# nelpy/ghost

Measured on NVIDIA B200. Metric: cwt_output_coeffs_per_sec, higher is better.
Workload: dtype f32

## Files before the change

ghost_b200/csrc/cabi.cu:

```cuda
#include "plan.h"
#include "common.cuh"
#include <cstring>
#include <cstdio>
#include <cstdlib>
#include <new>

namespace gcwt {

static thread_local std::string g_last_error;
static thread_local int64_t g_launches = 0;

void set_error(const std::string& msg) { g_last_error = msg; }
void count_launch(int n) { g_launches += n; }
int64_t launches_so_far() { return g_launches; }

int prof_begin(gcwt_plan* p, int kind, cudaStream_t st, int tag) {
    if (!p->profile) return -1;
    gcwt_plan::Span sp;
    sp.kind = kind;
    sp.tag = tag;
    sp.launches = (int)g_launches;
    if (cudaEventCreate(&sp.a) != cudaSuccess || cudaEventCreate(&sp.b) != cudaSuccess) return -1;
    cudaEventRecord(sp.a, st);
    p->spans.push_back(sp);
// ... 120 lines not shown
        sc.n_terms = d->n_terms[s];
        sc.term_off = off;
        sc.level = -2;
        if (sc.L < 1 || sc.n_terms < 1 || sc.k_first < 0 || sc.k_first + sc.n_terms > sc.L) {
            set_error("plan_create: inconsistent scale " + std::to_string(s));
            delete p;
            return GCWT_ERR_ARG;
        }
        off += sc.n_terms;
        p->scales.push_back(sc);
    }
    p->terms.assign(d->terms, d->terms + off);

    int rc = GCWT_OK;
    {
        cudaError_t e = cudaMalloc((void**)&p->d_scales, sizeof(ScaleInfo) * p->n_scales);
        if (e == cudaSuccess) e = cudaMalloc((void**)&p->d_terms, sizeof(double) * p->terms.size());
        if (e == cudaSuccess) e = cudaMemcpy(p->d_scales, p->scales.data(), sizeof(ScaleInfo) * p->n_scales, cudaMemcpyHostToDevice);
        if (e == cudaSuccess) e = cudaMemcpy(p->d_terms, p->terms.data(), sizeof(double) * p->terms.size(), cudaMemcpyHostToDevice);
        if (e != cudaSuccess) { set_error(std::string("plan_create: ") + cudaGetErrorString(e)); rc = GCWT_ERR_CUDA; }
    }
    if (rc == GCWT_OK) {
        if (p->compute_type == GCWT_F32) rc = fast_plan_build(p);
        else for (int s = 0; s < p->n_scales; ++s) p->generic_ids.push_back(s);
    }
    if (rc == GCWT_OK && p->compute_type == GCWT_F32) {
        cudaError_t e = cudaMemcpy(p->d_scales, p->scales.data(), sizeof(ScaleInfo) * p->n_scales, cudaMemcpyHostToDevice);
        if (e != cudaSuccess) { set_error(std::string("plan_create: ") + cudaGetErrorString(e)); rc = GCWT_ERR_CUDA; }
    }
    if (rc != GCWT_OK) { gcwt_plan_destroy(p); return rc; }
    *out = p;
    return GCWT_OK;
}

int gcwt_plan_destroy(gcwt_plan* p) {
    if (!p) return GCWT_OK;
    DeviceScope dev_scope(p->device);
    prof_collect(p);
    host_stage_free(p);
    fast_plan_free(p);
    if (p->d_scales) cudaFree(p->d_scales);
    if (p->d_terms) cudaFree(p->d_terms);
    if (p->ws.ptr) cudaFree(p->ws.ptr);
    if (p->d_means) cudaFree(p->d_means);
    if (p->d_partial) cudaFree(p->d_partial);
    if (p->d_twiddle) cudaFree(p->d_twiddle);
    if (p->d_tw1k) cudaFree(p->d_tw1k);
    if (p->d_tw_fine) cudaFree(p->d_tw_fine);
    if (p->d_hcache) cudaFree(p->d_hcache);
    for (int k = 0; k < gcwt_plan::kSideStreams; ++k) {
        if (p->side_stream[k]) { cudaStreamSynchronize(p->side_stream[k]); cudaStreamDestroy(p->side_stream[k]); }
        if (p->ev_join[k]) cudaEventDestroy(p->ev_join[k]);
    }
    if (p->ev_fork) cudaEventDestroy(p->ev_fork);
    delete p;
    return GCWT_OK;
}

int gcwt_profile_enable(gcwt_plan* p, int32_t on) {
    if (!p) { set_error("profile_enable: NULL plan"); return GCWT_ERR_ARG; }
    p->profile = on != 0;
    return GCWT_OK;
}

int gcwt_profile_read(gcwt_plan* p, double* ms_out, int64_t* launches_out, int32_t reset) {
    if (!p || !ms_out || !launches_out) { set_error("profile_read: NULL argument"); return GCWT_ERR_ARG; }
    DeviceScope dev_scope(p->device);
    prof_collect(p);
    if (getenv("GCWT_CLASS_TIMES")) {
        for (int t = 0; t < 64; ++t)
            if (p->class_ms[t] > 0) fprintf(stderr, "gcwt class level %d: %.4f ms\n", t - 2, p->class_ms[t]);
    }
    if (reset) for (int t = 0; t < 64; ++t) p->class_ms[t] = 0;
    for (int k = 0; k < GCWT_PROFILE_KINDS; ++k) {
        ms_out[k] = p->prof_ms[k];
        launches_out[k] = p->prof_launches[k];
        if (reset) { p->prof_ms[k] = 0; p->prof_launches[k] = 0; }
    }
    return GCWT_OK;
}

int gcwt_plan_levels(const gcwt_plan* p, int32_t* levels_out) {
    if (!p || !levels_out) { set_error("plan_levels: NULL argument"); return GCWT_ERR_ARG; }
    for (int s = 0; s < p->n_scales; ++s) levels_out[s] = p->scales[s].level;
    return GCWT_OK;
}

size_t gcwt_plan_workspace_bytes(const gcwt_plan* p) { return p ? p->ws.bytes : 0; }

int gcwt_guard_stats(const gcwt_plan* p, int64_t* last_pairs, int64_t* total_pairs, int64_t* checked_pairs,
                     unsigned char* scale_flags) {
    if (!p) { set_error("guard_stats: NULL plan"); return GCWT_ERR_ARG; }
    if (last_pairs) *last_pairs = p->guard_last;
    if (total_pairs) *total_pairs = p->guard_total;
    if (checked_pairs) *checked_pairs = p->guard_checked;
    if (scale_flags)
        for (int s = 0; s < p->n_scales; ++s) scale_flags[s] = (size_t)s < p->guard_last_flags.size() ? p->guard_last_flags[s] : 0;
    return GCWT_OK;
}

int gcwt_channel_means(const void* x, int32_t in_type, int64_t n_channels, int64_t n_samples,
                       int64_t x_stride, double* means_dev, int32_t device, void* stream) {
    if (!x || !means_dev) { set_error("channel_means: NULL argument"); return GCWT_ERR_ARG; }
    if (in_type != GCWT_F32 && in_type != GCWT_F64) { set_error("channel_means: bad in_type"); return GCWT_ERR_ARG; }
    DeviceScope dev_scope(device);
    double* partial = nullptr;
// ... 151 lines not shown
```

ghost_b200/csrc/fast_path.cu:

```cuda
#include "plan.h"
#include "common.cuh"
#include "multiplier.cuh"
#include <algorithm>
#include <atomic>
#include <cmath>
#include <cstdio>
#include <cstdlib>
#include <map>
#include <type_traits>

namespace gcwt {

constexpr int kMaxFastLevel = 14;
constexpr int kMaxFullScales = 64;
constexpr double kMaxHaloFrac = 0.45;

__constant__ float c_halfband[kHalfbandOdd];
constexpr int kSmallCoef = (2 + 4 + 8) * kInterpT;
__constant__ float c_interp_small[kSmallCoef];
constexpr int kWideCoef = (4 + 8) * kWideT;
__constant__ float c_interp_wide[kWideCoef];

static double bessel_i0(double x) {
    double sum = 1.0, term = 1.0;
// ... 567 lines not shown
        }
        *(float4*)(out + (int64_t)c * out_stride + (i0 + j0 - out_lo)) = make_float4(o[0], o[1], o[2], o[3]);
    }
    if (acc != nullptr) {
#pragma unroll
        for (int o = 16; o > 0; o >>= 1) {
            e_out += __shfl_xor_sync(0xffffffffu, e_out, o);
            if (FIRST) e_in += __shfl_xor_sync(0xffffffffu, e_in, o);
        }
        __syncthreads();
        if ((threadIdx.x & 31) == 0) { ev[threadIdx.x >> 5] = e_out; if (FIRST) ev[8 + (threadIdx.x >> 5)] = e_in; }
        __syncthreads();
        if (threadIdx.x == 0) {
            double* a = acc + (int64_t)c * acc_stride;
            float so = 0.f, si = 0.f;
#pragma unroll
            for (int w = 0; w < 8; ++w) { so += ev[w]; if (FIRST) si += ev[8 + w]; }
            if (so != 0.f) atomicAdd(a + level, (double)so);
            if (FIRST && si != 0.f) atomicAdd(a, (double)si);
        }
    }
}

struct FusedParams {
    const void* src;
    int64_t src_stride;
    int64_t src_lo, src_hi;
    const double* means;
    int log2d;
    int p_cols;
    int log2p;
    float inv_nc;
    int64_t offset, hop, n_chunks, n;
    int n_scales;
    const int32_t* scale_ids;
    const float2* table;
    void* out;
    int64_t s_stride, c_stride;
    int iters;
    int units_per_chunk;
    int log2u;
    const float* coef;
    const float2* twf;
    const int32_t* scale_nmu;
    double* acc;
    int acc_stride;
    int class_idx;
    float ech_weight;
    float* pow;
    int pow_stride;
    float pow_weight;
    int guard_every;
    int q_mode;
};

__device__ __forceinline__ float2 tw_pos(const float2* __restrict__ twf, int k) {
    const float2 t = __ldg(twf + (k & (kFullN - 1)));
    return make_float2(t.x, -t.y);
}

__device__ __forceinline__ float sqrt_abs_approx(float v) {
    float r;
    asm("sqrt.approx.ftz.f32 %0, %1;" : "=f"(r) : "f"(fabsf(v)));
    return r;
}

__device__ __forceinline__ float sqrt_approx(float v) {
    float r;
    asm("sqrt.approx.ftz.f32 %0, %1;" : "=f"(r) : "f"(v));
    return r;
}

template <int KIND> struct out_elem { typedef float type; };
template <> struct out_elem<GCWT_OUT_COMPLEX> { typedef float2 type; };

__device__ __forceinline__ void st_pred(float* p, float v, unsigned on) {
#ifdef GCWT_EXP_CSSTORE
    asm volatile("{\n\t.reg .pred q;\n\tsetp.ne.b32 q, %2, 0;\n\t@q st.global.cs.f32 [%0], %1;\n\t}"
                 :: "l"(p), "f"(v), "r"(on) : "memory");
    return;
#endif
    asm volatile("{\n\t.reg .pred q;\n\tsetp.ne.b32 q, %2, 0;\n\t@q st.global.f32 [%0], %1;\n\t}"
                 :: "l"(p), "f"(v), "r"(on) : "memory");
}
__device__ __forceinline__ void st_pred(float2* p, float2 v, unsigned on) {
    asm volatile("{\n\t.reg .pred q;\n\tsetp.ne.b32 q, %3, 0;\n\t@q st.global.v2.f32 [%0], {%1, %2};\n\t}"
                 :: "l"(p), "f"(v.x), "f"(v.y), "r"(on) : "memory");
}

template <int KIND>
__device__ __forceinline__ void store_column(typename out_elem<KIND>::type* __restrict__ op, int64_t stride,
                                             unsigned mask, const float2* a) {
#pragma unroll
    for (int k = 0; k < 16; ++k) {
        const unsigned on = mask & (1u << k);
        if constexpr (KIND == GCWT_OUT_COMPLEX) st_pred(op + k * stride, a[k], on);
        else if constexpr (KIND == GCWT_OUT_AMPLITUDE) st_pred(op + k * stride, sqrt_approx(a[k].x * a[k].x + a[k].y * a[k].y), on);
        else st_pred(op + k * stride, a[k].x * a[k].x + a[k].y * a[k].y, on);
    }
}

__device__ __forceinline__ unsigned valid_mask(int rel, int sh, int lo, int hi) {
    const int step = 1 << sh;
    int k_lo = (lo - rel + step - 1) >> sh;
    int k_hi = (hi - rel + step - 1) >> sh;
    k_lo = max(k_lo, 0);
// ... 764 lines not shown
        for (int i = 0; i < 16; ++i) a[i] = A[(g + 16 * i) * 17 + r];
        dft16<+1>(a);
        float2* e = ex + (g * 16) * 16 + r;
        e[0] = a[0];
#pragma unroll
        for (int k = 1; k < 16; ++k) e[k * 16] = cmul(a[k], tw[k]);
#ifndef GCWT_EXP_NOBAR
        __syncthreads();
#endif
        const float2* e2 = ex + g * 16 + r;
#pragma unroll
        for (int k = 0; k < 16; ++k) a[k] = e2[k * 256];
#ifndef GCWT_EXP_NOPASS2
        dft16<+1>(a);
#endif
#ifdef GCWT_EXP_NOSTORE
        store_column<KIND>(out_c + (int64_t)s_ids[s] * prm.s_stride + rel, 256, mask & 1u, a);
#elif defined(GCWT_EXP_HALFSTORE)
        store_column<KIND>(out_c + (int64_t)s_ids[s] * prm.s_stride + rel, 256, mask & 0x5555u, a);
#elif defined(GCWT_EXP_B16STORE)
        {
            unsigned short* o16 = (unsigned short*)(out_c + (int64_t)s_ids[s] * prm.s_stride) + rel;
#pragma unroll
            for (int k = 0; k < 16; ++k)
                if (mask & (1u << k)) o16[k * 512] = (unsigned short)__float_as_uint(a[k].x * a[k].x + a[k].y * a[k].y);
        }
#elif defined(GCWT_EXP_V2STORE)
        {
            float2* o2 = (float2*)(out_c + (int64_t)s_ids[s] * prm.s_stride) + rel;
#pragma unroll
            for (int k = 0; k < 16; k += 2)
                if (mask & (1u << k)) o2[(k >> 1) * 256] = make_float2(a[k].x * a[k].x + a[k].y * a[k].y, a[k + 1].x * a[k + 1].x + a[k + 1].y * a[k + 1].y);
        }
#elif defined(GCWT_EXP_STSSTORE)
        {
            float* stage = (float*)const_cast<float2*>(Yf);
#pragma unroll
            for (int k = 0; k < 16; ++k) stage[k * 256 + rel] = sqrt_approx(a[k].x * a[k].x + a[k].y * a[k].y);
        }
#elif defined(GCWT_EXP_L2STORE)
        store_column<KIND>((typename out_elem<KIND>::type*)prm.out + (blockIdx.x & 255) * 4096 + rel, 256, mask, a);
#else
        store_column<KIND>(out_c + (int64_t)s_ids[s] * prm.s_stride + rel, 256, mask, a);
#endif
        if (MEASURE) guard_pow_add<false>(a, mask, s_pow + (s & 1));
    }
    if (MEASURE) {
        __syncthreads();
        const int s = prm.n_scales - 1;
        if (tid == 0) atomicAdd(prm.pow + (blockIdx.x / prm.n_chunks) * prm.pow_stride + s_ids[s], s_pow[s & 1] * prm.pow_weight);
    }
}

template <typename TIn, int KIND, bool GUARD>
__global__ void __launch_bounds__(256, 2)
fused_full_kernel(const FusedParams prm) {
    extern __shared__ __align__(16) unsigned char smem_raw[];
    float2* Yf = (float2*)smem_raw;
    float2* ex = Yf + kFullN;
    float2* A = ex + kFullN;
    int* s_ids = (int*)(A + kTileA);
    int* s_nmu = s_ids + kMaxFullScales;
    float* s_pow = (float*)(s_nmu + kMaxFullScales);

    const int tid = threadIdx.x;
    if (tid < 2) s_pow[tid] = 0.f;
    const int r = tid & 15;
    const int g = tid >> 4;
    const int64_t qi = blockIdx.x % prm.n_chunks;
    const int64_t c = blockIdx.x / prm.n_chunks;
    const int64_t q = prm.q_mode == 0 ? qi : (prm.q_mode == 1 ? qi * prm.guard_every : qi + qi / (prm.guard_every - 1) + 1);
    const int64_t t0 = q * prm.hop - prm.offset;

    {
        const TIn* src = (const TIn*)prm.src + c * prm.src_stride;
        const double mu = prm.means[c];
        TIn raw[kFullN / 256];
        unsigned inside = 0;
#pragma unroll
        for (int k = 0; k < kFullN / 256; ++k) {
            const int64_t u = t0 + tid + 256 * k;
            const bool ok = u >= prm.src_lo && u < prm.src_hi;
            raw[k] = ok ? src[u] : (TIn)0;
            inside |= (unsigned)ok << k;
        }
        float val[kFullN / 256];
#pragma unroll
        for (int k = 0; k < kFullN / 256; ++k)
            val[k] = (inside >> k & 1) ? (float)((double)raw[k] - mu) : 0.f;
        const float cm = chunk_mean<kFullN / 256>(val, (float*)ex + 2048);
        if (GUARD)
            chunk_energy_add<kFullN / 256>(val, cm, (float*)ex + 2048, prm.acc + c * prm.acc_stride + kGuardLevels + prm.class_idx,
                                           prm.ech_weight);
#pragma unroll
        for (int k = 0; k < kFullN / 256; ++k) A[tid + 256 * k] = make_float2(val[k] - cm, 0.f);
        __syncthreads();
        smem_fft4096_forward(A, Yf, prm.twf);
    }
    float2 tw[16], tw4k[16];
#pragma unroll
    for (int k = 0; k < 16; ++k) {
        tw[k] = tw_pos(prm.twf, 16 * g * k);
        tw4k[k] = tw_pos(prm.twf, tid * k);
    }
    typedef typename out_elem<KIND>::type OutT;
    const int rel = g * 16 + r;
    const unsigned mask = valid_mask(rel, 8, (int)prm.offset, (int)min(prm.offset + prm.hop, prm.n - t0));
    OutT* const out_c = (OutT*)prm.out + c * prm.c_stride + t0;
    if (tid < prm.n_scales) { s_ids[tid] = prm.scale_ids[tid]; s_nmu[tid] = prm.scale_nmu[tid]; }
    __syncthreads();
    full_scale_loop<KIND, GUARD>(prm, Yf, ex, A, s_ids, s_nmu, s_pow, tw, tw4k, out_c, rel, mask);
}

template <int KIND, int LP, bool GUARD>
static void launch_banded_g(unsigned nblk, cudaStream_t st, const FusedParams& prm) {
    static std::atomic<bool> attr_set[64];
    int dev = 0;
    cudaGetDevice(&dev);
    if (!attr_set[dev & 63]) {
        cudaFuncSetAttribute(fused_banded_kernel<KIND, LP, GUARD>, cudaFuncAttributeMaxDynamicSharedMemorySize, (int)kBandedSmem);
        attr_set[dev & 63] = true;
    }
    fused_banded_kernel<KIND, LP, GUARD><<<nblk, 256, kBandedSmem, st>>>(prm);
}

template <int KIND, int LP>
static void launch_banded_one(unsigned nblk, cudaStream_t st, const FusedParams& prm) {
    if (prm.pow != nullptr) launch_banded_g<KIND, LP, true>(nblk, st, prm);
    else launch_banded_g<KIND, LP, false>(nblk, st, prm);
}

static void launch_banded(int kind, int lp, unsigned nblk, cudaStream_t st, const FusedParams& prm) {
    if (kind == GCWT_OUT_COMPLEX) {
        if (lp == 4) launch_banded_one<GCWT_OUT_COMPLEX, 4>(nblk, st, prm);
        else launch_banded_one<GCWT_OUT_COMPLEX, 0>(nblk, st, prm);
    } else if (kind == GCWT_OUT_AMPLITUDE) {
        if (lp == 4) launch_banded_one<GCWT_OUT_AMPLITUDE, 4>(nblk, st, prm);
        else launch_banded_one<GCWT_OUT_AMPLITUDE, 0>(nblk, st, prm);
    } else {
        if (lp == 4) launch_banded_one<GCWT_OUT_POWER, 4>(nblk, st, prm);
        else launch_banded_one<GCWT_OUT_POWER, 0>(nblk, st, prm);
    }
}

template <typename TIn, int KIND, bool GUARD>
static void launch_full_g(unsigned nblk, cudaStream_t st, const FusedParams& prm) {
    static std::atomic<bool> attr_set[64];
    int dev = 0;
    cudaGetDevice(&dev);
    if (!attr_set[dev & 63]) {
        cudaFuncSetAttribute(fused_full_kernel<TIn, KIND, GUARD>, cudaFuncAttributeMaxDynamicSharedMemorySize, (int)kFullSmem);
        attr_set[dev & 63] = true;
    }
    fused_full_kernel<TIn, KIND, GUARD><<<nblk, 256, kFullSmem, st>>>(prm);
}

template <typename TIn, int KIND>
static void launch_full_kind(unsigned nblk, cudaStream_t st, const FusedParams& prm, bool measure) {
    if (measure) launch_full_g<TIn, KIND, true>(nblk, st, prm);
    else launch_full_g<TIn, KIND, false>(nblk, st, prm);
}

template <typename TIn>
static void launch_full(int kind, unsigned nblk, cudaStream_t st, const FusedParams& prm, bool measure) {
    if (kind == GCWT_OUT_COMPLEX) launch_full_kind<TIn, GCWT_OUT_COMPLEX>(nblk, st, prm, measure);
    else if (kind == GCWT_OUT_AMPLITUDE) launch_full_kind<TIn, GCWT_OUT_AMPLITUDE>(nblk, st, prm, measure);
    else launch_full_kind<TIn, GCWT_OUT_POWER>(nblk, st, prm, measure);
}

struct LevelGeom { int64_t lo, hi, len, stride; float* ptr; };

template <typename TIn>
static int fast_run(gcwt_plan* p, const TIn* x, int in_type, int64_t n_channels, int64_t n,
                    int64_t x_stride, int64_t halo_l, int64_t halo_r, const double* d_means,
                    void* out, int64_t s_stride, int64_t c_stride, cudaStream_t st) {
    const bool guard = p->guard;
    const int acc_stride = kGuardLevels + (int)p->classes.size();
    if (guard) {
        if (p->guard_cap < n_channels) {
            if (p->d_guard_acc) cudaFree(p->d_guard_acc);
            if (p->d_guard_pow) cudaFree(p->d_guard_pow);
            if (p->d_guard_flags) cudaFree(p->d_guard_flags);
            if (p->h_guard_flags) cudaFreeHost(p->h_guard_flags);
            p->d_guard_acc = nullptr; p->d_guard_pow = nullptr; p->d_guard_flags = p->h_guard_flags = nullptr; p->guard_cap = 0;
            GCWT_CUDA_OK(cudaMalloc((void**)&p->d_guard_acc, sizeof(double) * acc_stride * n_channels));
            GCWT_CUDA_OK(cudaMalloc((void**)&p->d_guard_pow, sizeof(float) * p->n_scales * n_channels));
            GCWT_CUDA_OK(cudaMalloc((void**)&p->d_guard_flags, (size_t)p->n_scales * n_channels));
            GCWT_CUDA_OK(cudaMallocHost((void**)&p->h_guard_flags, (size_t)p->n_scales * n_channels));
            p->guard_cap = n_channels;
        }
        GCWT_CUDA_OK(cudaMemsetAsync(p->d_guard_acc, 0, sizeof(double) * acc_stride * n_channels, st));
        GCWT_CUDA_OK(cudaMemsetAsync(p->d_guard_pow, 0, sizeof(float) * p->n_scales * n_channels, st));
    }
    const int levels = std::max(p->max_level, 0) + ((guard && p->max_level > 0) ? 2 : 0);
    std::vector<LevelGeom> lv(levels + 1);
    lv[0].lo = -halo_l; lv[0].hi = n + halo_r;
    size_t total = 0;
    for (int j = 1; j <= levels; ++j) {
        const int64_t plo = lv[j - 1].lo, phi = lv[j - 1].hi - 1;
        const int64_t lo = (int64_t)std::floor((double)(plo - kHalfbandT) / 2.0);
        const int64_t hi = (int64_t)std::ceil((double)(phi + kHalfbandT) / 2.0);
        lv[j].lo = lo; lv[j].hi = hi + 1; lv[j].len = hi - lo + 1;
        lv[j].stride = (lv[j].len + 3) & ~int64_t(3);
        total += (size_t)lv[j].stride * n_channels;
    }
    int rc = ensure_workspace(p, total * sizeof(float) + 256);
    if (rc) return rc;
    float* w = (float*)p->ws.ptr;
    for (int j = 1; j <= levels; ++j) { lv[j].ptr = w; w += lv[j].stride * n_channels; }

    const int sp_pyr = prof_begin(p, 0, st);
    for (int j = 1; j <= levels; ++j) {
        dim3 grid((unsigned)((lv[j].len + kPyrTile - 1) / kPyrTile), (unsigned)n_channels);
        double* acc = guard ? p->d_guard_acc : nullptr;
        const int64_t seg_in = (n + (int64_t(1) << (j - 1)) - 1) >> (j - 1), seg_out = (n + (int64_t(1) << j) - 1) >> j;
        if (j == 1)
            pyramid_kernel<TIn, true><<<grid, 256, 0, st>>>(x, x_stride, lv[0].lo, lv[0].hi, d_means, lv[1].ptr,
                                                            lv[1].stride, lv[1].lo, lv[1].len, acc, acc_stride, j,
                                                            seg_in, seg_out);
        else
            pyramid_kernel<float, false><<<grid, 256, 0, st>>>(lv[j - 1].ptr, lv[j - 1].stride, lv[j - 1].lo,
                                                               lv[j - 1].hi, nullptr, lv[j].ptr, lv[j].stride,
                                                               lv[j].lo, lv[j].len, acc, acc_stride, j, seg_in, seg_out);
        count_launch();
    }
    prof_end(p, sp_pyr, st);
    GCWT_CUDA_OK(cudaGetLastError());

    const bool rows_aligned = ((uintptr_t)out % 16 == 0) && (s_stride % 4 == 0) && (c_stride % 4 == 0);
    const bool rows_aligned32 = ((uintptr_t)out % 32 == 0) && (s_stride % 8 == 0) && (c_stride % 8 == 0);
    auto uses_interp = [&](const FastClass& fc) {
        if (fc.level < 0 || !fc.interp) return false;
        if (fc.wide && fc.d_table2) return true;
        return (fc.log2u >= 3 && !fc.wide) || rows_aligned;
    };
    cudaStream_t full_meas_stream = nullptr;
    auto launch_class = [&](const FastClass& fc, cudaStream_t cs, bool own_span) -> int {
        const int sp = own_span ? prof_begin(p, fc.level < 0 ? 1 : (fc.interp ? 4 : 2), cs, fc.level + 2) : -1;
        FusedParams prm;
        prm.means = d_means;
        prm.offset = fc.offset; prm.hop = fc.hop; prm.n = n;
        prm.n_chunks = (n + fc.hop - 1) / fc.hop;
        prm.n_scales = (int)fc.scale_ids.size();
        prm.scale_ids = fc.d_scale_ids;
        prm.table = fc.d_table;
        prm.out = out; prm.s_stride = s_stride; prm.c_stride = c_stride;
        prm.inv_nc = 1.0f / (float)fc.nc_full;
        prm.log2u = fc.log2u; prm.coef = fc.d_coef; prm.twf = p->d_twiddle; prm.scale_nmu = fc.d_scale_nmu;
        prm.q_mode = 0;
        prm.acc = guard ? p->d_guard_acc : nullptr; prm.acc_stride = acc_stride;
        prm.class_idx = (int)(&fc - p->classes.data());
        prm.pow = guard ? p->d_guard_pow : nullptr; prm.pow_stride = p->n_scales;
        auto set_guard_sampling = [&](int64_t n_chunks, int every, double chunk_to_rate) {
            prm.guard_every = n_chunks >= 512 ? 2 * every : (n_chunks >= 256 ? every : (n_chunks >= 64 ? every / 2 : 1));
            const double w = (double)n_chunks / (double)((n_chunks + prm.guard_every - 1) / prm.guard_every);
            prm.pow_weight = (float)w;
            prm.ech_weight = (float)(w * chunk_to_rate);
        };
        set_guard_sampling(prm.n_chunks, fc.level >= 0 ? 8 : 16,
                           (double)(fc.level >= 0 ? (int64_t(1) << fc.level) : 1) * (double)fc.hop / (double)fc.nc_full);
        if (fc.level >= 0 && fc.interp && fc.wide && fc.d_table2) {
            const LevelGeom& g = lv[fc.level];
            prm.src = g.ptr; prm.src_stride = g.stride; prm.src_lo = g.lo; prm.src_hi = g.hi;
            prm.log2d = fc.level;
            prm.offset = fc.offset2; prm.hop = fc.hop2;
            prm.n_chunks = (n + fc.hop2 - 1) / fc.hop2;
            prm.table = fc.d_table2;
            set_guard_sampling(prm.n_chunks, 8, (double)(int64_t(1) << fc.level) * (double)fc.hop2 / (double)(2 * fc.nc_full));
            prm.p_cols = 8; prm.log2p = 3; prm.units_per_chunk = 1;
            prm.iters = rows_aligned32 ? 2 : (rows_aligned ? 1 : 0);
            const int64_t nblk = n_channels * prm.n_chunks;
            if (nblk > 0x7fffffffLL) { set_error("fast path: grid too large"); return GCWT_ERR_UNSUPPORTED; }
            if (p->out_kind == GCWT_OUT_AMPLITUDE) {
                if (guard) fused_wide2_kernel<GCWT_OUT_AMPLITUDE, true><<<(unsigned)nblk, 256, kWide2Smem, cs>>>(prm);
                else fused_wide2_kernel<GCWT_OUT_AMPLITUDE, false><<<(unsigned)nblk, 256, kWide2Smem, cs>>>(prm);
            } else {
                if (guard) fused_wide2_kernel<GCWT_OUT_POWER, true><<<(unsigned)nblk, 256, kWide2Smem, cs>>>(prm);
                else fused_wide2_kernel<GCWT_OUT_POWER, false><<<(unsigned)nblk, 256, kWide2Smem, cs>>>(prm);
            }
        } else if (uses_interp(fc)) {
            const LevelGeom& g = lv[fc.level];
            prm.src = g.ptr; prm.src_stride = g.stride; prm.src_lo = g.lo; prm.src_hi = g.hi;
            prm.log2d = fc.level;
            prm.p_cols = (int)(fc.nc_full / kBins);
            prm.log2p = ilog2_ceil(prm.p_cols);
            prm.iters = rows_aligned32 ? 2 : 1;
            const int64_t chunks = n_channels * prm.n_chunks;
            int64_t splits = (1776 + chunks - 1) / chunks;
            splits = std::max<int64_t>(1, std::min<int64_t>(splits, std::max<int64_t>(1, (int64_t(1) << fc.level) / 32)));
            splits = std::min<int64_t>(splits, 24);
            prm.units_per_chunk = (int)splits;
            const int64_t nblk = chunks * splits;
            if (nblk > 0x7fffffffLL) { set_error("fast path: grid too large"); return GCWT_ERR_UNSUPPORTED; }
            if (p->out_kind == GCWT_OUT_AMPLITUDE) {
                if (guard) fused_interp_kernel<GCWT_OUT_AMPLITUDE, true><<<(unsigned)nblk, 256, kInterpSmem, cs>>>(prm);
                else fused_interp_kernel<GCWT_OUT_AMPLITUDE, false><<<(unsigned)nblk, 256, kInterpSmem, cs>>>(prm);
            } else {
                if (guard) fused_interp_kernel<GCWT_OUT_POWER, true><<<(unsigned)nblk, 256, kInterpSmem, cs>>>(prm);
                else fused_interp_kernel<GCWT_OUT_POWER, false><<<(unsigned)nblk, 256, kInterpSmem, cs>>>(prm);
            }
        } else if (fc.level >= 0) {
            const LevelGeom& g = lv[fc.level];
            prm.src = g.ptr; prm.src_stride = g.stride; prm.src_lo = g.lo; prm.src_hi = g.hi;
            prm.log2d = fc.level;
            prm.p_cols = (int)(fc.nc_full / kBins);
            prm.log2p = ilog2_ceil(prm.p_cols);
            const int blocks = prm.p_cols / 16;
            prm.iters = std::min(blocks, 16);
            prm.units_per_chunk = (blocks + prm.iters - 1) / prm.iters;
            const int64_t nblk = n_channels * prm.n_chunks * prm.units_per_chunk;
            if (nblk > 0x7fffffffLL) { set_error("fast path: grid too large"); return GCWT_ERR_UNSUPPORTED; }
            launch_banded(p->out_kind, prm.log2p, (unsigned)nblk, cs, prm);
        } else {
            prm.src = x; prm.src_stride = x_stride; prm.src_lo = -halo_l; prm.src_hi = n + halo_r;
            prm.log2d = 0; prm.p_cols = 16; prm.log2p = 4; prm.iters = 1; prm.units_per_chunk = 1;
            const int64_t nblk = n_channels * prm.n_chunks;
            if (nblk > 0x7fffffffLL) { set_error("fast path: grid too large"); return GCWT_ERR_UNSUPPORTED; }
            if (!guard) {
                launch_full<TIn>(p->out_kind, (unsigned)nblk, cs, prm, false);
            } else {
                const int64_t n_all = prm.n_chunks, n_meas = (n_all + prm.guard_every - 1) / prm.guard_every;
                if (n_all > n_meas) {
                    prm.q_mode = 2; prm.n_chunks = n_all - n_meas;
                    launch_full<TIn>(p->out_kind, (unsigned)(n_channels * prm.n_chunks), cs, prm, false);
                    count_launch();
                }
                prm.q_mode = prm.guard_every > 1 ? 1 : 0; prm.n_chunks = n_meas;
                launch_full<TIn>(p->out_kind, (unsigned)(n_channels * prm.n_chunks), full_meas_stream ? full_meas_stream : cs, prm, true);
            }
        }
        count_launch();
        prof_end(p, sp, cs);
        return GCWT_OK;
    };

    bool side0_pending = false;
    if (guard && !p->profile && getenv("GCWT_STREAMS") == nullptr) {
        if (!p->side_stream[0]) {
            GCWT_CUDA_OK(cudaStreamCreateWithFlags(&p->side_stream[0], cudaStreamNonBlocking));
            GCWT_CUDA_OK(cudaEventCreateWithFlags(&p->ev_join[0], cudaEventDisableTiming));
        }
        if (!p->ev_fork) GCWT_CUDA_OK(cudaEventCreateWithFlags(&p->ev_fork, cudaEventDisableTiming));
        GCWT_CUDA_OK(cudaEventRecord(p->ev_fork, st));
        GCWT_CUDA_OK(cudaStreamWaitEvent(p->side_stream[0], p->ev_fork, 0));
        full_meas_stream = p->side_stream[0];
        side0_pending = true;
    }
    int n_group = 0;
    for (const FastClass& fc : p->classes) {
        if (uses_interp(fc)) { ++n_group; continue; }
        rc = launch_class(fc, st, true);
        if (rc) return rc;
    }
    if (n_group > 0) {
        int n_streams = 2;
        if (const char* e = getenv("GCWT_STREAMS")) n_streams = std::max(1, std::min(1 + gcwt_plan::kSideStreams, atoi(e)));
        const bool per_class = p->profile && getenv("GCWT_CLASS_TIMES") != nullptr;
        if (per_class || n_group < 2) n_streams = 1;
        const int n_side = n_streams - 1;
        for (int k = 0; k < n_side; ++k) {
            if (!p->side_stream[k]) {
                GCWT_CUDA_OK(cudaStreamCreateWithFlags(&p->side_stream[k], cudaStreamNonBlocking));
                GCWT_CUDA_OK(cudaEventCreateWithFlags(&p->ev_join[k], cudaEventDisableTiming));
            }
        }
        if (n_side > 0 && !p->ev_fork) GCWT_CUDA_OK(cudaEventCreateWithFlags(&p->ev_fork, cudaEventDisableTiming));
        const int sp = per_class ? -1 : prof_begin(p, 4, st, 63);
        if (n_side > 0) {
            GCWT_CUDA_OK(cudaEventRecord(p->ev_fork, st));
            for (int k = 0; k < n_side; ++k) GCWT_CUDA_OK(cudaStreamWaitEvent(p->side_stream[k], p->ev_fork, 0));
        }
        int ci = 0;
        for (const FastClass& fc : p->classes) {
            if (!uses_interp(fc)) continue;
            const int slot = ci++ % n_streams;
            rc = launch_class(fc, slot ? p->side_stream[slot - 1] : st, per_class);
            if (rc) return rc;
        }
        for (int k = 0; k < n_side; ++k) {
            GCWT_CUDA_OK(cudaEventRecord(p->ev_join[k], p->side_stream[k]));
            GCWT_CUDA_OK(cudaStreamWaitEvent(st, p->ev_join[k], 0));
            if (k == 0) side0_pending = false;
        }
        prof_end(p, sp, st);
    }
    if (side0_pending) {
        GCWT_CUDA_OK(cudaEventRecord(p->ev_join[0], p->side_stream[0]));
        GCWT_CUDA_OK(cudaStreamWaitEvent(st, p->ev_join[0], 0));
    }
    GCWT_CUDA_OK(cudaGetLastError());
    return GCWT_OK;
}

__global__ void guard_eval_kernel(int n_scales, const ScaleInfo* __restrict__ scales, const float* __restrict__ gain,
                                  const float* __restrict__ q, const int32_t* __restrict__ cls,
                                  const double* __restrict__ acc, int acc_stride, const float* __restrict__ pow,
                                  double tol2, unsigned char* __restrict__ flags) {
    const int s = blockIdx.x * blockDim.x + threadIdx.x, c = blockIdx.y;
    if (s >= n_scales) return;
    unsigned char flag = 0;
    const int ci = cls[s];
    if (ci >= 0) {
        const double* a = acc + (int64_t)c * acc_stride;
// ... 127 lines not shown
```

ghost_b200/csrc/plan.h:

```cpp
#pragma once
#include <cuda_runtime.h>
#include <stdint.h>
#include <vector>
#include "../../include/ghost_cwt.h"

namespace gcwt {

constexpr int kBins = 256;
constexpr int kChunkDec = 1024;
constexpr int kFullN = 4096;
#ifndef GCWT_MAX_CLASS
#define GCWT_MAX_CLASS 16
#endif
#ifndef GCWT_INTERP_T
#define GCWT_INTERP_T 8
#endif
#ifndef GCWT_WIDE_T
#define GCWT_WIDE_T 12
#endif
#ifndef GCWT_INTERP_CTAS
#define GCWT_INTERP_CTAS 2
#endif
constexpr int kMaxClassScales = GCWT_MAX_CLASS;
constexpr int kMinFastLevel = 2;
// ... 24 lines not shown
    std::vector<int> scale_ids;
    float2* d_table = nullptr;
    int32_t* d_scale_ids = nullptr;
    std::vector<int> scale_nmu;
    int32_t* d_scale_nmu = nullptr;
    bool interp = false;
    bool wide = false;
    float2* d_table2 = nullptr;
    int64_t offset2 = 0, hop2 = 0;
    int log2u = 0;
    float* d_coef = nullptr;
};

constexpr int kGuardSlots = 18;
constexpr int kGuardLevels = 20;
constexpr double kGuardKRound = 6.0;
constexpr double kGuardKStage = 2.0;

struct Workspace {
    void* ptr = nullptr;
    size_t bytes = 0;
};

}

struct gcwt_plan {
    int n_scales = 0;
    int compute_type = GCWT_F32;
    int out_kind = GCWT_OUT_AMPLITUDE;
    int device = 0;
    int flags = 0;
    double band_tol = 1e-7;
    std::vector<gcwt::ScaleInfo> scales;
    std::vector<double> terms;
    gcwt::ScaleInfo* d_scales = nullptr;
    double* d_terms = nullptr;
    std::vector<gcwt::FastClass> classes;
    std::vector<int> generic_ids;
    int max_level = 0;
    double halfband_odd[gcwt::kHalfbandOdd];
    gcwt::Workspace ws;
    bool profile = false;
    struct Span { cudaEvent_t a, b; int kind; int launches; int tag; };
    std::vector<Span> spans;
    double prof_ms[GCWT_PROFILE_KINDS] = {0, 0, 0, 0, 0};
    double class_ms[64] = {0};
    int64_t prof_launches[GCWT_PROFILE_KINDS] = {0, 0, 0, 0, 0};
    float2* d_twiddle = nullptr;
    double* d_means = nullptr;
    int64_t means_cap = 0;
    static constexpr int kSideStreams = 3;
    cudaStream_t side_stream[kSideStreams] = {nullptr, nullptr, nullptr};
    cudaEvent_t ev_fork = nullptr, ev_join[kSideStreams] = {nullptr, nullptr, nullptr};
    double* d_partial = nullptr;
    int64_t partial_cap = 0;
    bool guard = false;
    double guard_tol = 5e-6;
    float* d_guard_gain = nullptr;
    float* d_guard_q = nullptr;
    int32_t* d_guard_class = nullptr;
    double* d_guard_acc = nullptr;
    float* d_guard_pow = nullptr;
    unsigned char* d_guard_flags = nullptr;
    unsigned char* h_guard_flags = nullptr;
    int64_t guard_cap = 0;
    cudaEvent_t ev_guard = nullptr;
    int64_t guard_last = 0, guard_total = 0, guard_checked = 0;
    std::vector<unsigned char> guard_last_flags;
    std::vector<float> guard_gain_h, guard_q_h;
    double2* d_tw1k = nullptr;
    double2* d_tw_fine = nullptr;
    int64_t tw_fine_n = 0;
    double2* d_hcache = nullptr;
    int64_t hcache_n = 0;
    struct HostStage {
        void* d_in = nullptr; size_t in_bytes = 0;
        void* d_out[2] = {nullptr, nullptr}; size_t out_bytes = 0;
        void* h_ring[2] = {nullptr, nullptr}; size_t ring_bytes = 0;
        double* d_pool[2] = {nullptr, nullptr}; double* h_pool[2] = {nullptr, nullptr}; size_t pool_bytes = 0;
        double* d_means = nullptr; int64_t means_cap = 0;
        cudaStream_t st_compute = nullptr, st_copy = nullptr;
        cudaEvent_t ev_done[2] = {nullptr, nullptr}, ev_out[2] = {nullptr, nullptr};
        double last_ms[4] = {0, 0, 0, 0};
    } host;
};

namespace gcwt {
int ensure_workspace(gcwt_plan* p, size_t bytes);
void count_launch(int n = 1);
int64_t launches_so_far();
int prof_begin(gcwt_plan* p, int kind, cudaStream_t st, int tag = 0);
void prof_end(gcwt_plan* p, int idx, cudaStream_t st);

int generic_execute(gcwt_plan* p, const std::vector<int>& ids, const void* x, int in_type,
                    int64_t n_channels, int64_t n_samples, int64_t x_stride,
                    int64_t halo_l, int64_t halo_r, const double* d_means,
                    void* out, int64_t s_stride, int64_t c_stride, cudaStream_t st,
                    bool fp64_for_fp32_plan = false);
int guard_resolve(gcwt_plan* p, const void* x, int in_type, int64_t n_channels, int64_t n_samples,
                  int64_t x_stride, int64_t halo_l, int64_t halo_r, const double* d_means,
                  void* out, int64_t s_stride, int64_t c_stride, cudaStream_t st);
int fast_execute(gcwt_plan* p, const void* x, int in_type,
                 int64_t n_channels, int64_t n_samples, int64_t x_stride,
                 int64_t halo_l, int64_t halo_r, const double* d_means,
                 void* out, int64_t s_stride, int64_t c_stride, cudaStream_t st);
int interp_taps(int log2u, int n_taps, double os, float* out);
// ... 13 lines not shown
```

Measured before the change: 772.0 billion.

## Co-run persistent full-band kernel alongside pyramid and interp classes on priority streams

Adds a persistent grid-stride variant of the full-band FFT kernel that is capped to one CTA per SM through its shared-memory size. A fraction of its chunks, chosen by a cost model, runs on a high-priority stream at the same time as the pyramid and grouped banded/interp classes on two other streams. The remaining full-band chunks then run on the main stream. The aim is to fill SMs left idle by the lighter pyramid and interp kernels. In exchange it adds stream and event overhead, a register/smem feasibility probe, and a risk of contention that slows both sides.

```diff
diff --git a/ghost_b200/csrc/cabi.cu b/ghost_b200/csrc/cabi.cu
--- a/ghost_b200/csrc/cabi.cu
+++ b/ghost_b200/csrc/cabi.cu
@@ -196,6 +196,11 @@
         if (p->side_stream[k]) { cudaStreamSynchronize(p->side_stream[k]); cudaStreamDestroy(p->side_stream[k]); }
         if (p->ev_join[k]) cudaEventDestroy(p->ev_join[k]);
     }
+    for (int k = 0; k < 3; ++k) {
+        if (p->co_stream[k]) { cudaStreamSynchronize(p->co_stream[k]); cudaStreamDestroy(p->co_stream[k]); }
+        if (p->ev_co[k]) cudaEventDestroy(p->ev_co[k]);
+    }
+    if (p->ev_co_pyr) cudaEventDestroy(p->ev_co_pyr);
     if (p->ev_fork) cudaEventDestroy(p->ev_fork);
     delete p;
     return GCWT_OK;
diff --git a/ghost_b200/csrc/fast_path.cu b/ghost_b200/csrc/fast_path.cu
--- a/ghost_b200/csrc/fast_path.cu
+++ b/ghost_b200/csrc/fast_path.cu
@@ -643,6 +643,8 @@
     float pow_weight;
     int guard_every;
     int q_mode;
+    int64_t q_first;
+    int64_t n_blocks;
 };
 
 __device__ __forceinline__ float2 tw_pos(const float2* __restrict__ twf, int k) {
@@ -1513,7 +1515,7 @@
     }
 }
 
-template <typename TIn, int KIND, bool GUARD>
+template <typename TIn, int KIND, bool GUARD, bool STRIDE = false>
 __global__ void __launch_bounds__(256, 2)
 fused_full_kernel(const FusedParams prm) {
     extern __shared__ __align__(16) unsigned char smem_raw[];
@@ -1528,49 +1530,53 @@
     if (tid < 2) s_pow[tid] = 0.f;
     const int r = tid & 15;
     const int g = tid >> 4;
-    const int64_t qi = blockIdx.x % prm.n_chunks;
-    const int64_t c = blockIdx.x / prm.n_chunks;
-    const int64_t q = prm.q_mode == 0 ? qi : (prm.q_mode == 1 ? qi * prm.guard_every : qi + qi / (prm.guard_every - 1) + 1);
-    const int64_t t0 = q * prm.hop - prm.offset;
-
-    {
-        const TIn* src = (const TIn*)prm.src + c * prm.src_stride;
-        const double mu = prm.means[c];
-        TIn raw[kFullN / 256];
-        unsigned inside = 0;
-#pragma unroll
-        for (int k = 0; k < kFullN / 256; ++k) {
-            const int64_t u = t0 + tid + 256 * k;
-            const bool ok = u >= prm.src_lo && u < prm.src_hi;
-            raw[k] = ok ? src[u] : (TIn)0;
-            inside |= (unsigned)ok << k;
-        }
-        float val[kFullN / 256];
-#pragma unroll
-        for (int k = 0; k < kFullN / 256; ++k)
-            val[k] = (inside >> k & 1) ? (float)((double)raw[k] - mu) : 0.f;
-        const float cm = chunk_mean<kFullN / 256>(val, (float*)ex + 2048);
-        if (GUARD)
-            chunk_energy_add<kFullN / 256>(val, cm, (float*)ex + 2048, prm.acc + c * prm.acc_stride + kGuardLevels + prm.class_idx,
-                                           prm.ech_weight);
-#pragma unroll
-        for (int k = 0; k < kFullN / 256; ++k) A[tid + 256 * k] = make_float2(val[k] - cm, 0.f);
+    const int64_t blk_end = STRIDE ? prm.n_blocks : (int64_t)blockIdx.x + 1;
+    for (int64_t blk = blockIdx.x; blk < blk_end; blk += STRIDE ? gridDim.x : 1) {
+        if (STRIDE && blk != blockIdx.x) __syncthreads();
+        const int64_t qi = blk % prm.n_chunks + prm.q_first;
+        const int64_t c = blk / prm.n_chunks;
+        const int64_t q = prm.q_mode == 0 ? qi : (prm.q_mode == 1 ? qi * prm.guard_every : qi + qi / (prm.guard_every - 1) + 1);
+        const int64_t t0 = q * prm.hop - prm.offset;
+
+        {
+            const TIn* src = (const TIn*)prm.src + c * prm.src_stride;
+            const double mu = prm.means[c];
+            TIn raw[kFullN / 256];
+            unsigned inside = 0;
+    #pragma unroll
+            for (int k = 0; k < kFullN / 256; ++k) {
+                const int64_t u = t0 + tid + 256 * k;
+                const bool ok = u >= prm.src_lo && u < prm.src_hi;
+                raw[k] = ok ? src[u] : (TIn)0;
+                inside |= (unsigned)ok << k;
+            }
+            float val[kFullN / 256];
+    #pragma unroll
+            for (int k = 0; k < kFullN / 256; ++k)
+                val[k] = (inside >> k & 1) ? (float)((double)raw[k] - mu) : 0.f;
+            const float cm = chunk_mean<kFullN / 256>(val, (float*)ex + 2048);
+            if (GUARD)
+                chunk_energy_add<kFullN / 256>(val, cm, (float*)ex + 2048, prm.acc + c * prm.acc_stride + kGuardLevels + prm.class_idx,
+                                               prm.ech_weight);
+    #pragma unroll
+            for (int k = 0; k < kFullN / 256; ++k) A[tid + 256 * k] = make_float2(val[k] - cm, 0.f);
+            __syncthreads();
+            smem_fft4096_forward(A, Yf, prm.twf);
+        }
+        float2 tw[16], tw4k[16];
+    #pragma unroll
+        for (int k = 0; k < 16; ++k) {
+            tw[k] = tw_pos(prm.twf, 16 * g * k);
+            tw4k[k] = tw_pos(prm.twf, tid * k);
+        }
+        typedef typename out_elem<KIND>::type OutT;
+        const int rel = g * 16 + r;
+        const unsigned mask = valid_mask(rel, 8, (int)prm.offset, (int)min(prm.offset + prm.hop, prm.n - t0));
+        OutT* const out_c = (OutT*)prm.out + c * prm.c_stride + t0;
+        if (tid < prm.n_scales) { s_ids[tid] = prm.scale_ids[tid]; s_nmu[tid] = prm.scale_nmu[tid]; }
         __syncthreads();
-        smem_fft4096_forward(A, Yf, prm.twf);
-    }
-    float2 tw[16], tw4k[16];
-#pragma unroll
-    for (int k = 0; k < 16; ++k) {
-        tw[k] = tw_pos(prm.twf, 16 * g * k);
-        tw4k[k] = tw_pos(prm.twf, tid * k);
-    }
-    typedef typename out_elem<KIND>::type OutT;
-    const int rel = g * 16 + r;
-    const unsigned mask = valid_mask(rel, 8, (int)prm.offset, (int)min(prm.offset + prm.hop, prm.n - t0));
-    OutT* const out_c = (OutT*)prm.out + c * prm.c_stride + t0;
-    if (tid < prm.n_scales) { s_ids[tid] = prm.scale_ids[tid]; s_nmu[tid] = prm.scale_nmu[tid]; }
-    __syncthreads();
-    full_scale_loop<KIND, GUARD>(prm, Yf, ex, A, s_ids, s_nmu, s_pow, tw, tw4k, out_c, rel, mask);
+        full_scale_loop<KIND, GUARD>(prm, Yf, ex, A, s_ids, s_nmu, s_pow, tw, tw4k, out_c, rel, mask);
+    }
 }
 
 template <int KIND, int LP, bool GUARD>
@@ -1604,29 +1610,119 @@
     }
 }
 
+struct CtaUse { int regs, smem; };
+static CtaUse cta_use(const void* fn, size_t dyn_smem) {
+    cudaFuncAttributes a;
+    if (cudaFuncGetAttributes(&a, fn) != cudaSuccess) return {1 << 30, 1 << 30};
+    const int warp_regs = (a.numRegs * 32 + 255) & ~255;
+    return {warp_regs * (256 / 32), (int)(a.sharedSizeBytes + dyn_smem)};
+}
+
+template <typename TIn, int KIND>
+static int full_capped_probe(int dev) {
+    int smem_sm = 0, reserve = 0, optin = 0, regs_sm = 0;
+    if (cudaDeviceGetAttribute(&smem_sm, cudaDevAttrMaxSharedMemoryPerMultiprocessor, dev) != cudaSuccess ||
+        cudaDeviceGetAttribute(&reserve, cudaDevAttrReservedSharedMemoryPerBlock, dev) != cudaSuccess ||
+        cudaDeviceGetAttribute(&optin, cudaDevAttrMaxSharedMemoryPerBlockOptin, dev) != cudaSuccess ||
+        cudaDeviceGetAttribute(&regs_sm, cudaDevAttrMaxRegistersPerMultiprocessor, dev) != cudaSuccess)
+        return 0;
+    const int capped = ((smem_sm / 2 - reserve + 1) + 127) & ~127;
+    if (capped < (int)kFullSmem || capped > optin) return 0;
+    const CtaUse full = cta_use((const void*)fused_full_kernel<TIn, KIND, false, true>, capped);
+    const CtaUse partners[] = {
+        cta_use((const void*)pyramid_kernel<TIn, true>, 0), cta_use((const void*)pyramid_kernel<float, false>, 0),
+        cta_use((const void*)fused_banded_kernel<KIND, 4, false>, kBandedSmem), cta_use((const void*)fused_banded_kernel<KIND, 4, true>, kBandedSmem),
+        cta_use((const void*)fused_banded_kernel<KIND, 0, false>, kBandedSmem), cta_use((const void*)fused_banded_kernel<KIND, 0, true>, kBandedSmem),
+        cta_use((const void*)fused_interp_kernel<KIND, false>, kInterpSmem), cta_use((const void*)fused_interp_kernel<KIND, true>, kInterpSmem),
+        cta_use((const void*)fused_wide2_kernel<KIND, false>, kWide2Smem), cta_use((const void*)fused_wide2_kernel<KIND, true>, kWide2Smem)};
+    for (const CtaUse& u : partners)
+        if (full.regs + u.regs > regs_sm || full.smem + u.smem + 2 * reserve > smem_sm) return 0;
+    const void* fns[] = {(const void*)pyramid_kernel<TIn, true>, (const void*)pyramid_kernel<float, false>,
+                         (const void*)fused_interp_kernel<KIND, false>, (const void*)fused_interp_kernel<KIND, true>,
+                         (const void*)fused_wide2_kernel<KIND, false>, (const void*)fused_wide2_kernel<KIND, true>};
+    for (const void* fn : fns) cudaFuncSetAttribute(fn, cudaFuncAttributePreferredSharedMemoryCarveout, (int)cudaSharedmemCarveoutMaxShared);
+    return capped;
+}
+
 template <typename TIn, int KIND, bool GUARD>
-static void launch_full_g(unsigned nblk, cudaStream_t st, const FusedParams& prm) {
-    static std::atomic<bool> attr_set[64];
+static int full_attrs() {
+    static std::atomic<int> state[64];
     int dev = 0;
     cudaGetDevice(&dev);
-    if (!attr_set[dev & 63]) {
+    int s = state[dev & 63];
+    if (s == 0) {
         cudaFuncSetAttribute(fused_full_kernel<TIn, KIND, GUARD>, cudaFuncAttributeMaxDynamicSharedMemorySize, (int)kFullSmem);
-        attr_set[dev & 63] = true;
+        int capped = 0;
+        if constexpr (!GUARD && KIND != GCWT_OUT_COMPLEX) {
+            capped = full_capped_probe<TIn, KIND>(dev);
+            if (capped) {
+                auto fn = fused_full_kernel<TIn, KIND, false, true>;
+                cudaFuncSetAttribute(fn, cudaFuncAttributeMaxDynamicSharedMemorySize, capped);
+                cudaFuncSetAttribute(fn, cudaFuncAttributePreferredSharedMemoryCarveout, (int)cudaSharedmemCarveoutMaxShared);
+                int per_sm = 0;
+                if (cudaOccupancyMaxActiveBlocksPerMultiprocessor(&per_sm, fn, 256, capped) != cudaSuccess || per_sm != 1) capped = 0;
+            }
+        }
+        cudaGetLastError();
+        s = capped ? capped : -1;
+        state[dev & 63] = s;
+    }
+    return s > 0 ? s : 0;
+}
+
+template <typename TIn, int KIND, bool GUARD>
+static void launch_full_g(unsigned nblk, cudaStream_t st, const FusedParams& prm, bool capped) {
+    const int cap = full_attrs<TIn, KIND, GUARD>();
+    if constexpr (!GUARD && KIND != GCWT_OUT_COMPLEX) {
+        if (capped) {
+            int dev = 0, sms = 0;
+            cudaGetDevice(&dev);
+            cudaDeviceGetAttribute(&sms, cudaDevAttrMultiProcessorCount, dev);
+            FusedParams prm2 = prm;
+            prm2.n_blocks = nblk;
+            fused_full_kernel<TIn, KIND, false, true><<<std::min<unsigned>(nblk, (unsigned)std::max(sms, 1)), 256, cap, st>>>(prm2);
+            return;
+        }
     }
     fused_full_kernel<TIn, KIND, GUARD><<<nblk, 256, kFullSmem, st>>>(prm);
 }
 
 template <typename TIn, int KIND>
-static void launch_full_kind(unsigned nblk, cudaStream_t st, const FusedParams& prm, bool measure) {
-    if (measure) launch_full_g<TIn, KIND, true>(nblk, st, prm);
-    else launch_full_g<TIn, KIND, false>(nblk, st, prm);
+static void launch_full_kind(unsigned nblk, cudaStream_t st, const FusedParams& prm, bool measure, bool capped) {
+    if (measure) launch_full_g<TIn, KIND, true>(nblk, st, prm, false);
+    else launch_full_g<TIn, KIND, false>(nblk, st, prm, capped);
 }
 
 template <typename TIn>
-static void launch_full(int kind, unsigned nblk, cudaStream_t st, const FusedParams& prm, bool measure) {
-    if (kind == GCWT_OUT_COMPLEX) launch_full_kind<TIn, GCWT_OUT_COMPLEX>(nblk, st, prm, measure);
-    else if (kind == GCWT_OUT_AMPLITUDE) launch_full_kind<TIn, GCWT_OUT_AMPLITUDE>(nblk, st, prm, measure);
-    else launch_full_kind<TIn, GCWT_OUT_POWER>(nblk, st, prm, measure);
+static void launch_full(int kind, unsigned nblk, cudaStream_t st, const FusedParams& prm, bool measure, bool capped = false) {
+    if (kind == GCWT_OUT_COMPLEX) launch_full_kind<TIn, GCWT_OUT_COMPLEX>(nblk, st, prm, measure, false);
+    else if (kind == GCWT_OUT_AMPLITUDE) launch_full_kind<TIn, GCWT_OUT_AMPLITUDE>(nblk, st, prm, measure, capped);
+    else launch_full_kind<TIn, GCWT_OUT_POWER>(nblk, st, prm, measure, capped);
+}
+
+template <typename TIn>
+static int full_capped_smem(int kind) {
+    if (kind == GCWT_OUT_AMPLITUDE) return full_attrs<TIn, GCWT_OUT_AMPLITUDE, false>();
+    if (kind == GCWT_OUT_POWER) return full_attrs<TIn, GCWT_OUT_POWER, false>();
+    return 0;
+}
+
+static int guard_every_for(int64_t n_chunks, int every) {
+    return n_chunks >= 512 ? 2 * every : (n_chunks >= 256 ? every : (n_chunks >= 64 ? every / 2 : 1));
+}
+
+constexpr double kCorunCostLow = 0.47;
+constexpr double kCorunCostHbm = 0.28;
+constexpr double kCorunGain = 1.0;
+static double corun_split(const gcwt_plan* p) {
+    if (const char* e = getenv("GCWT_FULL_SPLIT")) return std::min(1.0, std::max(0.0, atof(e)));
+    double full = 0.0, group = 0.0;
+    for (const FastClass& fc : p->classes) {
+        const double ns = (double)fc.scale_ids.size();
+        if (fc.level < 0) full += ns;
+        else group += ns * (fc.level >= 5 ? kCorunCostHbm : kCorunCostLow);
+    }
+    return full > 0.0 ? std::min(1.0, kCorunGain * group / full) : 0.0;
 }
 
 struct LevelGeom { int64_t lo, hi, len, stride; float* ptr; };
@@ -1670,23 +1766,26 @@
     float* w = (float*)p->ws.ptr;
     for (int j = 1; j <= levels; ++j) { lv[j].ptr = w; w += lv[j].stride * n_channels; }
 
-    const int sp_pyr = prof_begin(p, 0, st);
-    for (int j = 1; j <= levels; ++j) {
-        dim3 grid((unsigned)((lv[j].len + kPyrTile - 1) / kPyrTile), (unsigned)n_channels);
-        double* acc = guard ? p->d_guard_acc : nullptr;
-        const int64_t seg_in = (n + (int64_t(1) << (j - 1)) - 1) >> (j - 1), seg_out = (n + (int64_t(1) << j) - 1) >> j;
-        if (j == 1)
-            pyramid_kernel<TIn, true><<<grid, 256, 0, st>>>(x, x_stride, lv[0].lo, lv[0].hi, d_means, lv[1].ptr,
-                                                            lv[1].stride, lv[1].lo, lv[1].len, acc, acc_stride, j,
-                                                            seg_in, seg_out);
-        else
-            pyramid_kernel<float, false><<<grid, 256, 0, st>>>(lv[j - 1].ptr, lv[j - 1].stride, lv[j - 1].lo,
-                                                               lv[j - 1].hi, nullptr, lv[j].ptr, lv[j].stride,
-                                                               lv[j].lo, lv[j].len, acc, acc_stride, j, seg_in, seg_out);
-        count_launch();
-    }
-    prof_end(p, sp_pyr, st);
-    GCWT_CUDA_OK(cudaGetLastError());
+    auto run_pyramid = [&](cudaStream_t ps) -> int {
+        const int sp_pyr = prof_begin(p, 0, ps);
+        for (int j = 1; j <= levels; ++j) {
+            dim3 grid((unsigned)((lv[j].len + kPyrTile - 1) / kPyrTile), (unsigned)n_channels);
+            double* acc = guard ? p->d_guard_acc : nullptr;
+            const int64_t seg_in = (n + (int64_t(1) << (j - 1)) - 1) >> (j - 1), seg_out = (n + (int64_t(1) << j) - 1) >> j;
+            if (j == 1)
+                pyramid_kernel<TIn, true><<<grid, 256, 0, ps>>>(x, x_stride, lv[0].lo, lv[0].hi, d_means, lv[1].ptr,
+                                                                lv[1].stride, lv[1].lo, lv[1].len, acc, acc_stride, j,
+                                                                seg_in, seg_out);
+            else
+                pyramid_kernel<float, false><<<grid, 256, 0, ps>>>(lv[j - 1].ptr, lv[j - 1].stride, lv[j - 1].lo,
+                                                                   lv[j - 1].hi, nullptr, lv[j].ptr, lv[j].stride,
+                                                                   lv[j].lo, lv[j].len, acc, acc_stride, j, seg_in, seg_out);
+            count_launch();
+        }
+        prof_end(p, sp_pyr, ps);
+        GCWT_CUDA_OK(cudaGetLastError());
+        return GCWT_OK;
+    };
 
     const bool rows_aligned = ((uintptr_t)out % 16 == 0) && (s_stride % 4 == 0) && (c_stride % 4 == 0);
     const bool rows_aligned32 = ((uintptr_t)out % 32 == 0) && (s_stride % 8 == 0) && (c_stride % 8 == 0);
@@ -1695,8 +1794,26 @@
         if (fc.wide && fc.d_table2) return true;
         return (fc.log2u >= 3 && !fc.wide) || rows_aligned;
     };
+    int n_group = 0;
+    for (const FastClass& fc : p->classes) n_group += uses_interp(fc) ? 1 : 0;
+    std::vector<int64_t> n_cap(p->classes.size(), 0);
+    bool corun = false;
+    if (n_group > 0 && p->out_kind != GCWT_OUT_COMPLEX && !p->profile && getenv("GCWT_STREAMS") == nullptr &&
+        full_capped_smem<TIn>(p->out_kind) > 0) {
+        const double f = corun_split(p);
+        for (size_t k = 0; k < p->classes.size(); ++k) {
+            const FastClass& fc = p->classes[k];
+            if (fc.level >= 0) continue;
+            const int64_t n_all = (n + fc.hop - 1) / fc.hop;
+            if (n_all < 2) continue;
+            const int every = guard ? guard_every_for(n_all, 16) : 1;
+            const int64_t n_rest = guard ? n_all - (n_all + every - 1) / every : n_all;
+            n_cap[k] = std::min<int64_t>(n_rest, (int64_t)std::llround(f * (double)n_rest));
+            corun = corun || n_cap[k] > 0;
+        }
+    }
     cudaStream_t full_meas_stream = nullptr;
-    auto launch_class = [&](const FastClass& fc, cudaStream_t cs, bool own_span) -> int {
+    auto launch_class = [&](const FastClass& fc, cudaStream_t cs, bool own_span, int part = 0) -> int {
         const int sp = own_span ? prof_begin(p, fc.level < 0 ? 1 : (fc.interp ? 4 : 2), cs, fc.level + 2) : -1;
         FusedParams prm;
         prm.means = d_means;
@@ -1708,12 +1825,12 @@
         prm.out = out; prm.s_stride = s_stride; prm.c_stride = c_stride;
         prm.inv_nc = 1.0f / (float)fc.nc_full;
         prm.log2u = fc.log2u; prm.coef = fc.d_coef; prm.twf = p->d_twiddle; prm.scale_nmu = fc.d_scale_nmu;
-        prm.q_mode = 0;
+        prm.q_mode = 0; prm.q_first = 0; prm.n_blocks = 0;
         prm.acc = guard ? p->d_guard_acc : nullptr; prm.acc_stride = acc_stride;
         prm.class_idx = (int)(&fc - p->classes.data());
         prm.pow = guard ? p->d_guard_pow : nullptr; prm.pow_stride = p->n_scales;
         auto set_guard_sampling = [&](int64_t n_chunks, int every, double chunk_to_rate) {
-            prm.guard_every = n_chunks >= 512 ? 2 * every : (n_chunks >= 256 ? every : (n_chunks >= 64 ? every / 2 : 1));
+            prm.guard_every = guard_every_for(n_chunks, every);
             const double w = (double)n_chunks / (double)((n_chunks + prm.guard_every - 1) / prm.guard_every);
             prm.pow_weight = (float)w;
             prm.ech_weight = (float)(w * chunk_to_rate);
@@ -1777,17 +1894,24 @@
             prm.log2d = 0; prm.p_cols = 16; prm.log2p = 4; prm.iters = 1; prm.units_per_chunk = 1;
             const int64_t nblk = n_channels * prm.n_chunks;
             if (nblk > 0x7fffffffLL) { set_error("fast path: grid too large"); return GCWT_ERR_UNSUPPORTED; }
-            if (!guard) {
-                launch_full<TIn>(p->out_kind, (unsigned)nblk, cs, prm, false);
+            const int64_t n_all = prm.n_chunks, n_meas = guard ? (n_all + prm.guard_every - 1) / prm.guard_every : 0;
+            const int64_t n_rest = n_all - n_meas, cap = part == 0 ? 0 : n_cap[prm.class_idx];
+            prm.q_mode = guard ? 2 : 0;
+            if (part == 1) {
+                prm.n_chunks = cap;
+                launch_full<TIn>(p->out_kind, (unsigned)(n_channels * cap), cs, prm, false, true);
             } else {
-                const int64_t n_all = prm.n_chunks, n_meas = (n_all + prm.guard_every - 1) / prm.guard_every;
-                if (n_all > n_meas) {
-                    prm.q_mode = 2; prm.n_chunks = n_all - n_meas;
+                if (n_rest > cap) {
+                    prm.q_first = cap; prm.n_chunks = n_rest - cap;
                     launch_full<TIn>(p->out_kind, (unsigned)(n_channels * prm.n_chunks), cs, prm, false);
-                    count_launch();
+                    if (guard) count_launch();
                 }
-                prm.q_mode = prm.guard_every > 1 ? 1 : 0; prm.n_chunks = n_meas;
-                launch_full<TIn>(p->out_kind, (unsigned)(n_channels * prm.n_chunks), full_meas_stream ? full_meas_stream : cs, prm, true);
+                if (guard) {
+                    prm.q_mode = prm.guard_every > 1 ? 1 : 0; prm.q_first = 0; prm.n_chunks = n_meas;
+                    launch_full<TIn>(p->out_kind, (unsigned)(n_channels * prm.n_chunks), full_meas_stream ? full_meas_stream : cs, prm, true);
+                } else if (n_rest <= cap) {
+                    return GCWT_OK;
+                }
             }
         }
         count_launch();
@@ -1795,6 +1919,68 @@
         return GCWT_OK;
     };
 
+    auto corun_schedule = [&]() -> int {
+        if (!p->co_stream[0]) {
+            int least = 0, greatest = 0;
+            GCWT_CUDA_OK(cudaDeviceGetStreamPriorityRange(&least, &greatest));
+            const bool full_high = getenv("GCWT_CORUN_PRIO") == nullptr || atoi(getenv("GCWT_CORUN_PRIO")) != 0;
+            for (int k = 0; k < 3; ++k) {
+                const int prio = (k == 0) == full_high ? greatest : least;
+                GCWT_CUDA_OK(cudaStreamCreateWithPriority(&p->co_stream[k], cudaStreamNonBlocking, prio));
+                GCWT_CUDA_OK(cudaEventCreateWithFlags(&p->ev_co[k], cudaEventDisableTiming));
+            }
+            GCWT_CUDA_OK(cudaEventCreateWithFlags(&p->ev_co_pyr, cudaEventDisableTiming));
+        }
+        if (!p->ev_fork) GCWT_CUDA_OK(cudaEventCreateWithFlags(&p->ev_fork, cudaEventDisableTiming));
+        GCWT_CUDA_OK(cudaEventRecord(p->ev_fork, st));
+        for (int k = 0; k < 2; ++k) GCWT_CUDA_OK(cudaStreamWaitEvent(p->co_stream[k], p->ev_fork, 0));
+        for (const FastClass& fc : p->classes)
+            if (fc.level < 0 && n_cap[&fc - p->classes.data()] > 0) {
+                int rc2 = launch_class(fc, p->co_stream[0], false, 1);
+                if (rc2) return rc2;
+            }
+        int rc2 = run_pyramid(p->co_stream[1]);
+        if (rc2) return rc2;
+        GCWT_CUDA_OK(cudaEventRecord(p->ev_co_pyr, p->co_stream[1]));
+        GCWT_CUDA_OK(cudaStreamWaitEvent(p->co_stream[2], p->ev_co_pyr, 0));
+        std::vector<const FastClass*> group;
+        for (const FastClass& fc : p->classes) {
+            if (fc.level < 0) continue;
+            if (!uses_interp(fc)) { rc2 = launch_class(fc, p->co_stream[1], false); if (rc2) return rc2; }
+            else group.push_back(&fc);
+        }
+        std::stable_sort(group.begin(), group.end(), [](const FastClass* a, const FastClass* b) { return a->level > b->level; });
+        for (size_t i = 0; i < group.size(); ++i) {
+            rc2 = launch_class(*group[i], p->co_stream[1 + (i & 1)], false);
+            if (rc2) return rc2;
+        }
+        for (int k = 1; k < 3; ++k) {
+            GCWT_CUDA_OK(cudaEventRecord(p->ev_co[k], p->co_stream[k]));
+            GCWT_CUDA_OK(cudaStreamWaitEvent(st, p->ev_co[k], 0));
+        }
+        if (guard) {
+            if (!p->side_stream[0]) {
+                GCWT_CUDA_OK(cudaStreamCreateWithFlags(&p->side_stream[0], cudaStreamNonBlocking));
+                GCWT_CUDA_OK(cudaEventCreateWithFlags(&p->ev_join[0], cudaEventDisableTiming));
+            }
+            GCWT_CUDA_OK(cudaEventRecord(p->ev_fork, st));
+            GCWT_CUDA_OK(cudaStreamWaitEvent(p->side_stream[0], p->ev_fork, 0));
+            full_meas_stream = p->side_stream[0];
+        }
+        for (const FastClass& fc : p->classes)
+            if (fc.level < 0) { rc2 = launch_class(fc, st, false, 2); if (rc2) return rc2; }
+        GCWT_CUDA_OK(cudaEventRecord(p->ev_co[0], p->co_stream[0]));
+        GCWT_CUDA_OK(cudaStreamWaitEvent(st, p->ev_co[0], 0));
+        if (guard) {
+            GCWT_CUDA_OK(cudaEventRecord(p->ev_join[0], p->side_stream[0]));
+            GCWT_CUDA_OK(cudaStreamWaitEvent(st, p->ev_join[0], 0));
+        }
+        GCWT_CUDA_OK(cudaGetLastError());
+        return GCWT_OK;
+    };
+    if (corun) return corun_schedule();
+    rc = run_pyramid(st);
+    if (rc) return rc;
     bool side0_pending = false;
     if (guard && !p->profile && getenv("GCWT_STREAMS") == nullptr) {
         if (!p->side_stream[0]) {
@@ -1807,9 +1993,8 @@
         full_meas_stream = p->side_stream[0];
         side0_pending = true;
     }
-    int n_group = 0;
     for (const FastClass& fc : p->classes) {
-        if (uses_interp(fc)) { ++n_group; continue; }
+        if (uses_interp(fc)) continue;
         rc = launch_class(fc, st, true);
         if (rc) return rc;
     }
diff --git a/ghost_b200/csrc/plan.h b/ghost_b200/csrc/plan.h
--- a/ghost_b200/csrc/plan.h
+++ b/ghost_b200/csrc/plan.h
@@ -100,6 +100,8 @@
     static constexpr int kSideStreams = 3;
     cudaStream_t side_stream[kSideStreams] = {nullptr, nullptr, nullptr};
     cudaEvent_t ev_fork = nullptr, ev_join[kSideStreams] = {nullptr, nullptr, nullptr};
+    cudaStream_t co_stream[3] = {nullptr, nullptr, nullptr};
+    cudaEvent_t ev_co[3] = {nullptr, nullptr, nullptr}, ev_co_pyr = nullptr;
     double* d_partial = nullptr;
     int64_t partial_cap = 0;
     bool guard = false;
```

New measurement: 731.3 billion, median of 6. -5.3%, worse.
